# fab-jul/imgcomp-cvpr

Hardware: AMD Instinct MI355X
Metric: Megapixels/s encode+pc-logits (and decode) per node (higher is better)
Workload: dtype f32

## Files before the change

imgcomp_cvpr_amd/csrc/conv_mfma.hip:

```cpp
#include "internal.h"

typedef float f32x16 __attribute__((ext_vector_type(16)));
typedef float f32x4 __attribute__((ext_vector_type(4)));

#define GKC 8

struct GArgs {
    const float* x; const float* scale; const float* shift; float* y;
    int N, IH, IW;
    int GH, GW;
    int OH, OW, OS;
    int Cout, relu;
    int tiles_x, tiles_y;
    int ncot;
    unsigned long long* prof;
};

__global__ void pack_conv_mfma_kernel(const float* __restrict__ w, float* __restrict__ out, int KW, int Cin, int Cout,
                                      int transposed, int NTY, int NTX, int NCOT, int kyb, int kys, int kxb, int kxs,
                                      int total) {
    const int idx = blockIdx.x * 256 + threadIdx.x;
    if (idx >= total) return;
    const int j = idx & 3, l = (idx >> 2) & 63;
    int r = idx >> 8;
    const int n = r % NCOT; r /= NCOT;
    const int NT = NTY * NTX;
    const int t = r % NT, c = r / NT;
    const int ty = t / NTX, tx = t % NTX;
    const int ky = kyb + kys * ty, kx = kxb + kxs * tx;
    const int ci = GKC * c + 2 * j + (l >> 5), co = 32 * n + (l & 31);
    float v = 0.f;
    if (co < Cout)
        v = transposed ? w[(((size_t)ky * KW + kx) * Cout + co) * Cin + ci]
                       : w[(((size_t)ky * KW + kx) * Cin + ci) * Cout + co];
    out[idx] = v;
}

struct GPhase { const float* wp; int oy0, ox0, py, px; };

template <int NTY, int NTX, int PS, int WK, int TR, int TC, int CPC = 1>
struct GGeo {
    static constexpr int ROWS = (TR - 1) * PS + NTY, COLS = (TC - 1) * PS + NTX;
    static constexpr int S = COLS, CS = ROWS * COLS, CHUNK = GKC * WK * CS * CPC;
    static constexpr int NST = (CHUNK + 255) / 256;
    static constexpr int LDSF = 2 * NST * 256;
    static_assert(NST <= 32, "in-bounds mask is 32 bits");
};

template <int NTY, int NTX, int PS, int CIN, int WM, int WN, int WK, int PT, int TR, int TC, int RD, bool KEEP = false, bool X1 = false, int CPC = 1>
__device__ __forceinline__ void conv_mfma_body(const GArgs& a, const GPhase& ph, float* __restrict__ lds, f32x16* keep = nullptr) {
#ifdef CM_PROF
    const unsigned long long cm_t0 = __builtin_amdgcn_s_memtime();
#endif
    using G = GGeo<NTY, NTX, PS, WK, TR, TC, CPC>;
    constexpr int NT = NTY * NTX;
    constexpr int NCH = CIN / (GKC * WK * CPC);
    static_assert(CPC == 1 || WK == 1, "several channel groups per chunk: whole-K waves only");
    static_assert(CIN % (GKC * WK * CPC) == 0, "Cin multiple of the chunk");
    constexpr int S = G::S, CS = G::CS, CHUNK = G::CHUNK, NST = G::NST;
    static_assert(WM * WN * WK == 4, "4 waves per work-group");
    static_assert(TR * TC == 32 * PT * WN, "tile = PT accumulator tiles per wave x WN pixel groups");
    static_assert(NT % RD == 0 && RD >= 3, "ring depth must divide the tap count");
    static_assert(CIN % (GKC * WK) == 0, "Cin multiple of 8 * WK");
    static_assert(WK == 1 || (16 % WK == 0 && WM * WN * WK * PT * 16 * 64 <= G::LDSF), "reduction scratch fits in the staging buffers");

    const int tid = threadIdx.x, lane = tid & 63, wave = tid >> 6;
    const int wm = wave % WM, wn = (wave / WM) % WN, wk = wave / (WM * WN);
    int b = ic_xcd_run(blockIdx.x, gridDim.x);
    const int tx_ = b % a.tiles_x; b /= a.tiles_x;
    const int ty_ = b % a.tiles_y; const int n = b / a.tiles_y;
    const int cot = blockIdx.y * WM + wm;
    const int ncot = a.ncot;
    const int gx0 = tx_ * TC, gy0 = ty_ * TR;
    const int IHW = a.IH * a.IW;
    const float* __restrict__ xin = a.x + (size_t)n * CIN * IHW;

    int goff[NST];
    unsigned inb = 0;
    const int iy0 = gy0 * PS + ph.oy0, ix0 = gx0 * PS + ph.ox0;
#pragma unroll
    for (int i = 0; i < NST; ++i) {
        const int e = tid + 256 * i;
        const int ci = e / CS, rem = e - ci * CS;
        const int rr = rem / S, cc = rem - rr * S;
        const int iy = iy0 + rr, ix = ix0 + cc;
        const bool ok = (e < CHUNK) && iy >= 0 && iy < a.IH && ix >= 0 && ix < a.IW;
        goff[i] = ok ? ci * IHW + iy * a.IW + ix : 0;
        inb |= (ok ? 1u : 0u) << i;
    }
    const int j = lane & 31, kh = lane >> 5;
    int boff[PT];
#pragma unroll
    for (int p = 0; p < PT; ++p) {
        const int q = 32 * (PT * wn + p) + j;
        boff[p] = (GKC * wk + kh) * CS + (q / TC) * PS * S + (q % TC) * PS;
    }
    const int cot_u = __builtin_amdgcn_readfirstlane(cot), wk_u = __builtin_amdgcn_readfirstlane(wk);
    const __amdgpu_buffer_rsrc_t wr = __builtin_amdgcn_make_buffer_rsrc(
        (void*)ph.wp, 0, (CIN / GKC) * NT * ncot * 256 * 4, 0x00020000);
    const unsigned wlane = (unsigned)lane * 16u;
    const int wstep = ncot * 1024;
    const int cstep = NT * wstep;
    auto wload = [&](int c8, int t) -> f32x4 {
        return __builtin_bit_cast(f32x4, __builtin_amdgcn_raw_buffer_load_b128(wr, wlane, c8 * cstep + t * wstep + cot_u * 1024, 0));
    };

    f32x16 acc[PT];
#pragma unroll
    for (int p = 0; p < PT; ++p)
#pragma unroll
        for (int r = 0; r < 16; ++r) acc[p][r] = 0.f;

    constexpr int RPW = 16 / WK;
    float bsc[RPW], bsh[RPW];
    {
        const __amdgpu_buffer_rsrc_t scr = __builtin_amdgcn_make_buffer_rsrc((void*)a.scale, 0, a.Cout * 4, 0x00020000);
        const __amdgpu_buffer_rsrc_t shr = __builtin_amdgcn_make_buffer_rsrc((void*)a.shift, 0, a.Cout * 4, 0x00020000);
#pragma unroll
        for (int rr = 0; rr < RPW; ++rr) {
            const int r = (WK > 1 ? wk * RPW : 0) + rr;
            const unsigned co4 = (unsigned)(32 * cot + (r & 3) + 8 * (r >> 2) + 4 * (lane >> 5)) * 4u;
            bsc[rr] = __builtin_bit_cast(float, __builtin_amdgcn_raw_buffer_load_b32(scr, co4, 0, 0));
            bsh[rr] = __builtin_bit_cast(float, __builtin_amdgcn_raw_buffer_load_b32(shr, co4, 0, 0));
        }
    }
    f32x4 ring[RD];
#pragma unroll
    for (int t = 0; t < RD - 2; ++t) ring[t] = wload(wk_u, t);
    static_assert(!X1 || (PT == 1 && WM == 1 && WN == 1), "extra channel: one pixel tile per wave");
    const int cotx_u = X1 ? (a.Cout - 1) / 32 : 0;
    const unsigned xlane = (unsigned)(lane >> 5) * 512u;
    auto xload = [&](int c8, int t) -> f32x4 {
        return __builtin_bit_cast(f32x4, __builtin_amdgcn_raw_buffer_load_b128(wr, xlane, c8 * cstep + t * wstep + cotx_u * 1024, 0));
    };
    f32x4 xring[X1 ? RD : 1];
    float accx = 0.f;
    if constexpr (X1) {
#pragma unroll
        for (int t = 0; t < RD - 2; ++t) xring[t] = xload(wk_u, t);
    }
#pragma unroll
    for (int i = 0; i < NST; ++i) {
        const float v = xin[goff[i]];
        lds[tid + 256 * i] = ((inb >> i) & 1) ? v : 0.f;
    }
    __syncthreads();
#ifdef CM_PROF
    const unsigned long long cm_t1 = __builtin_amdgcn_s_memtime();
#endif

    for (int c = 0; c < NCH; ++c) {
        const bool more = c + 1 < NCH;
        float st[NST];
        if (more) {
            const float* xc = xin + (size_t)(c + 1) * GKC * WK * CPC * IHW;
#pragma unroll
            for (int i = 0; i < NST; ++i) st[i] = xc[goff[i]];
        }
        const float* __restrict__ L = lds + (c & 1) * (NST * 256);
        const int c8 = c * WK * CPC + wk_u, c8n = more ? (c + 1) * WK * CPC + wk_u : c8;
        constexpr int NU = CPC * NT;
        float bq[2][4][PT];
#pragma unroll
        for (int ks = 0; ks < 4; ++ks)
#pragma unroll
            for (int p = 0; p < PT; ++p) bq[0][ks][p] = L[boff[p] + 2 * ks * CS];
#pragma unroll
        for (int u = 0; u < NU; ++u) {
            {
                const int un = u + RD - 2;
                if (un < NU) ring[un % RD] = wload(c8 + un / NT, un % NT);
                else ring[un % RD] = wload(c8n + (un - NU) / NT, (un - NU) % NT);
                if constexpr (X1) {
                    if (un < NU) xring[un % RD] = xload(c8 + un / NT, un % NT);
                    else xring[un % RD] = xload(c8n + (un - NU) / NT, (un - NU) % NT);
                }
            }
            if (u + 1 < NU) {
                const int tn = (u + 1) % NT, gn = (u + 1) / NT;
                const int tapoff = (tn / NTX) * S + (tn % NTX) + 8 * gn * CS;
#pragma unroll
                for (int ks = 0; ks < 4; ++ks)
#pragma unroll
                    for (int p = 0; p < PT; ++p) bq[(u + 1) & 1][ks][p] = L[boff[p] + 2 * ks * CS + tapoff];
            }
#pragma unroll
            for (int ks = 0; ks < 4; ++ks) {
                const float av = ring[u % RD][ks];
#pragma unroll
                for (int p = 0; p < PT; ++p)
                    acc[p] = __builtin_amdgcn_mfma_f32_32x32x2f32(av, bq[u & 1][ks][p], acc[p], 0, 0, 0);
                if constexpr (X1) asm volatile("v_fmac_f32 %0, %1, %2" : "+v"(accx) : "v"(xring[u % RD][ks]), "v"(bq[u & 1][ks][0]));
            }
#pragma unroll
            for (int i = 0; i < 4 * PT; ++i) {
                __builtin_amdgcn_sched_group_barrier(0x008, 1, 0);
                if (i == 0) __builtin_amdgcn_sched_group_barrier(0x020, 1, 0);
                if (X1 && i == 1) __builtin_amdgcn_sched_group_barrier(0x020, 1, 0);
                if (X1) __builtin_amdgcn_sched_group_barrier(0x002, 1, 0);
                if (u + 1 < NU) __builtin_amdgcn_sched_group_barrier(0x100, 1, 0);
            }
            __builtin_amdgcn_sched_barrier(0);
        }
        if (more) {
            float* __restrict__ Ln = lds + ((c & 1) ^ 1) * (NST * 256);
#pragma unroll
            for (int i = 0; i < NST; ++i) Ln[tid + 256 * i] = ((inb >> i) & 1) ? st[i] : 0.f;
        }
        asm volatile("s_waitcnt lgkmcnt(0)" ::: "memory");
        __builtin_amdgcn_s_barrier();
    }

#ifdef CM_PROF
    const unsigned long long cm_t2 = __builtin_amdgcn_s_memtime();
#endif
    float* __restrict__ y = a.y;
    const size_t OHW = (size_t)a.OH * a.OW;
    const size_t cbase = ((size_t)n * a.Cout + 32 * cot + 4 * kh) * OHW;
    if (WK > 1) {
        float* red = lds + (size_t)((wm * WN + wn) * WK) * (PT * 16 * 64);
#pragma unroll
        for (int p = 0; p < PT; ++p)
#pragma unroll
            for (int r = 0; r < 16; ++r) red[(size_t)((wk * PT + p) * 16 + r) * 64 + lane] = acc[p][r];
        __syncthreads();
#pragma unroll
        for (int p = 0; p < PT; ++p)
#pragma unroll
            for (int rr = 0; rr < RPW; ++rr) {
                const int r = wk * RPW + rr;
                float sum = 0.f;
#pragma unroll
                for (int k2 = 0; k2 < WK; ++k2) sum += red[(size_t)((k2 * PT + p) * 16 + r) * 64 + lane];
                acc[p][rr] = sum;
            }
    }
    if constexpr (X1) {
        const float half_sum = accx + __shfl_xor(accx, 32);
        if (WK > 1) {
            __syncthreads();
            if (lane < 32) lds[wk * 32 + lane] = half_sum;
            __syncthreads();
        }
        if (wk == 0 && lane < 32) {
            float sum = WK > 1 ? 0.f : half_sum;
            if (WK > 1) {
#pragma unroll
                for (int k2 = 0; k2 < WK; ++k2) sum += lds[k2 * 32 + lane];
            }
            const int cx = a.Cout - 1;
            const int q = lane, gy = gy0 + q / TC, gx = gx0 + q % TC;
            if (gy < a.GH && gx < a.GW) {
                float v = fmaf(sum, a.scale[cx], a.shift[cx]);
                if (a.relu) v = fmaxf(v, 0.f);
                y[((size_t)n * a.Cout + cx) * OHW + (size_t)(gy * a.OS + ph.py) * a.OW + (gx * a.OS + ph.px)] = v;
            }
        }
    }
    if constexpr (KEEP) {
        static_assert(!KEEP || WK == 1, "paired phases: whole-K waves");
#pragma unroll
        for (int p = 0; p < PT; ++p)
#pragma unroll
            for (int r = 0; r < 16; ++r) {
                float v = fmaf(acc[p][r], bsc[r], bsh[r]);
                keep[p][r] = a.relu ? fmaxf(v, 0.f) : v;
            }
        return;
    }
#pragma unroll
    for (int p = 0; p < PT; ++p) {
        const int q = 32 * (PT * wn + p) + j;
        const int gy = gy0 + q / TC, gx = gx0 + q % TC;
        if (gy < a.GH && gx < a.GW) {
            const size_t pix = cbase + (size_t)(gy * a.OS + ph.py) * a.OW + (gx * a.OS + ph.px);
#pragma unroll
            for (int rr = 0; rr < RPW; ++rr) {
                const int r = (WK > 1 ? wk * RPW : 0) + rr;
                const int crow = (r & 3) + 8 * (r >> 2);
                const int co = 32 * cot + crow + 4 * kh;
                if (co < (X1 ? a.Cout - 1 : a.Cout)) {
                    float v = fmaf(acc[p][rr], bsc[rr], bsh[rr]);
                    if (a.relu) v = fmaxf(v, 0.f);
                    y[pix + (size_t)crow * OHW] = v;
                }
            }
        }
    }
#ifdef CM_PROF
    if (a.prof && lane == 0) {
        unsigned long long* d = a.prof + 4 * (((size_t)blockIdx.y * gridDim.x + blockIdx.x) * 4 + wave);
        d[0] = cm_t0; d[1] = cm_t1; d[2] = cm_t2; d[3] = __builtin_amdgcn_s_memtime();
    }
#endif
}

template <int NTY, int NTX, int PS, int CIN, int WM, int WN, int WK, int PT, int TR, int TC, int RD, int CPC = 1>
__global__ __launch_bounds__(256) void conv_mfma_kernel(const GArgs a, const GPhase ph) {
    __shared__ float lds[GGeo<NTY, NTX, PS, WK, TR, TC, CPC>::LDSF];
    conv_mfma_body<NTY, NTX, PS, CIN, WM, WN, WK, PT, TR, TC, RD, false, false, CPC>(a, ph, lds);
}

template <int NTY, int NTX, int PS, int CIN, int WM, int WN, int WK, int PT, int TR, int TC, int RD>
__global__ __launch_bounds__(256) void conv_mfma_x1_kernel(const GArgs a, const GPhase ph) {
    __shared__ float lds[GGeo<NTY, NTX, PS, WK, TR, TC>::LDSF];
    conv_mfma_body<NTY, NTX, PS, CIN, WM, WN, WK, PT, TR, TC, RD, false, true>(a, ph, lds);
}

struct GPhases4 { GPhase p[4]; };
template <int CIN, int WM, int WN, int PT, int TR, int TC>
__global__ __launch_bounds__(256) void deconv5_mfma_kernel(const GArgs a, const GPhases4 ph) {
    __shared__ float lds[GGeo<3, 3, 1, 1, TR, TC>::LDSF];
    switch (blockIdx.z) {
        case 0: conv_mfma_body<2, 2, 1, CIN, WM, WN, 1, PT, TR, TC, 4>(a, ph.p[0], lds); break;
        case 1: conv_mfma_body<2, 3, 1, CIN, WM, WN, 1, PT, TR, TC, 3>(a, ph.p[1], lds); break;
        case 2: conv_mfma_body<3, 2, 1, CIN, WM, WN, 1, PT, TR, TC, 3>(a, ph.p[2], lds); break;
        default: conv_mfma_body<3, 3, 1, CIN, WM, WN, 1, PT, TR, TC, 3>(a, ph.p[3], lds); break;
    }
}

typedef float f32x2g __attribute__((ext_vector_type(2)));
template <int CIN, int WM, int WN, int PT, int TR, int TC, int CPC>
__global__ __launch_bounds__(256) void deconv5_pair_kernel(const GArgs a, const GPhases4 ph) {
    __shared__ float lds[GGeo<3, 3, 1, 1, TR, TC, CPC>::LDSF];
    f32x16 v0[PT], v1[PT];
    const int py = blockIdx.z;
    if (py == 0) {
        conv_mfma_body<2, 2, 1, CIN, WM, WN, 1, PT, TR, TC, 4, true, false, CPC>(a, ph.p[0], lds, v0);
        conv_mfma_body<2, 3, 1, CIN, WM, WN, 1, PT, TR, TC, 3, true, false, CPC>(a, ph.p[1], lds, v1);
    } else {
        conv_mfma_body<3, 2, 1, CIN, WM, WN, 1, PT, TR, TC, 3, true, false, CPC>(a, ph.p[2], lds, v0);
        conv_mfma_body<3, 3, 1, CIN, WM, WN, 1, PT, TR, TC, 3, true, false, CPC>(a, ph.p[3], lds, v1);
    }
    const int lane = threadIdx.x & 63, wave = threadIdx.x >> 6;
    const int wm = wave % WM, wn = (wave / WM) % WN;
    int b = ic_xcd_run(blockIdx.x, gridDim.x);
    const int tx_ = b % a.tiles_x; b /= a.tiles_x;
    const int ty_ = b % a.tiles_y; const int n = b / a.tiles_y;
    const int cot = blockIdx.y * WM + wm;
    const int j = lane & 31, kh = lane >> 5;
    const size_t OHW = (size_t)a.OH * a.OW;
    float* __restrict__ y = a.y + ((size_t)n * a.Cout + 32 * cot + 4 * kh) * OHW;
#pragma unroll
    for (int p = 0; p < PT; ++p) {
        const int q = 32 * (PT * wn + p) + j;
        const int gy = ty_ * TR + q / TC, gx = tx_ * TC + q % TC;
        if (gy < a.GH && gx < a.GW) {
            const size_t pix = (size_t)(gy * 2 + py) * a.OW + gx * 2;
#pragma unroll
            for (int r = 0; r < 16; ++r) {
                const int crow = (r & 3) + 8 * (r >> 2);
                if (32 * cot + crow + 4 * kh < a.Cout)
                    *(f32x2g*)(y + pix + (size_t)crow * OHW) = f32x2g{v0[p][r], v1[p][r]};
            }
        }
    }
}

static unsigned long long* g_cm_prof = nullptr;
#ifdef CM_PROF
extern "C" void ic_conv2d_mfma_set_prof(unsigned lo, unsigned hi) { g_cm_prof = (unsigned long long*)(((unsigned long long)hi << 32) | lo); }
#endif
static int ncot_for(int Cout) { return ic_cdiv(Cout, 32) <= 2 ? 2 : ic_cdiv(ic_cdiv(Cout, 32), 4) * 4; }

static void phase_taps(int K, int pad, int p, int* nt, int* o0, int* kb) {
    const int k0 = (p + pad) & 1;
    const int cnt = (K - k0 + 1) / 2;
    const int kmax = k0 + 2 * (cnt - 1);
    *nt = cnt;
    *o0 = (p + pad - kmax) / 2;
    *kb = kmax;
}

static bool supported(int KH, int KW, int Cin, int Cout, int stride, int transposed) {
    if (KH == 3 && KW == 3 && stride == 2 && !transposed) return Cin == 128 && Cout <= 128;
    if (KH != 5 || KW != 5 || stride != 2) return false;
    if (!transposed) return (Cin == 64 && Cout == 128) || (Cin == 128 && Cout <= 128);
    return Cin == 128 && Cout == 64;
}

extern "C" size_t ic_conv2d_mfma_packed_floats(int KH, int KW, int Cin, int Cout, int stride, int transposed) {
    if (!supported(KH, KW, Cin, Cout, stride, transposed)) return 0;
    return (size_t)(Cin / GKC) * KH * KW * ncot_for(Cout) * 256;
}

extern "C" int ic_pack_conv2d_mfma_f32(const float* w_tf, float* w_packed, int KH, int KW, int Cin, int Cout,
                                       int stride, int transposed, ic_stream_t stream) {
    IC_CHECK_ARG(w_tf && w_packed);
    if (!supported(KH, KW, Cin, Cout, stride, transposed)) return IC_ERR_UNSUPPORTED;
    const int ncot = ncot_for(Cout), nch = Cin / GKC;
    hipStream_t st = (hipStream_t)stream;
    if (!transposed) {
        const int total = nch * KH * KW * ncot * 256;
        hipLaunchKernelGGL(pack_conv_mfma_kernel, dim3(ic_cdiv(total, 256)), dim3(256), 0, st, w_tf, w_packed, KW, Cin,
                           Cout, 0, KH, KW, ncot, 0, 1, 0, 1, total);
    } else {
        const int pad = 1;
        size_t off = 0;
        for (int py = 0; py < 2; ++py)
            for (int px = 0; px < 2; ++px) {
                int nty, ntx, oy0, ox0, kyb, kxb;
                phase_taps(KH, pad, py, &nty, &oy0, &kyb);
                phase_taps(KW, pad, px, &ntx, &ox0, &kxb);
                const int total = nch * nty * ntx * ncot * 256;
                hipLaunchKernelGGL(pack_conv_mfma_kernel, dim3(ic_cdiv(total, 256)), dim3(256), 0, st, w_tf,
                                   w_packed + off, KW, Cin, Cout, 1, nty, ntx, ncot, kyb, -2, kxb, -2, total);
                off += (size_t)total;
            }
    }
    IC_LAUNCH_CHECK();
    return IC_OK;
}

extern "C" int ic_conv2d_mfma_bn_act_f32(const float* x, const float* w_packed, const float* scale, const float* shift,
                                         float* y, int N, int Cin, int H, int W, int Cout, int KH, int KW, int stride,
                                         int transposed, int relu, ic_stream_t stream) {
    IC_CHECK_ARG(x && w_packed && scale && shift && y && N > 0 && H > 0 && W > 0);
    if (!supported(KH, KW, Cin, Cout, stride, transposed)) return IC_ERR_UNSUPPORTED;
    if ((long long)Cin * H * W >= (1ll << 31)) return IC_ERR_UNSUPPORTED;
    hipStream_t st = (hipStream_t)stream;
    const int ncot = ncot_for(Cout);
    GArgs a{};
    a.x = x; a.scale = scale; a.shift = shift; a.y = y;
    a.N = N; a.IH = H; a.IW = W; a.Cout = Cout; a.relu = relu; a.prof = g_cm_prof; a.ncot = ncot;
    if (!transposed) {
        GPhase ph{};
        ph.wp = w_packed; ph.py = 0; ph.px = 0;
        ph.oy0 = -ic_same_pad_before(H, KH, 2); ph.ox0 = -ic_same_pad_before(W, KW, 2);
        a.GH = ic_cdiv(H, 2); a.GW = ic_cdiv(W, 2); a.OH = a.GH; a.OW = a.GW; a.OS = 1;
        if (KH == 3) {
            a.tiles_x = ic_cdiv(a.GW, 16); a.tiles_y = ic_cdiv(a.GH, 2);
            hipLaunchKernelGGL((conv_mfma_kernel<3, 3, 2, 128, 1, 1, 4, 1, 2, 16, 3>),
                               dim3(a.tiles_x * a.tiles_y * N, ic_cdiv(Cout, 32)), dim3(256), 0, st, a, ph);
        } else if (Cin == 64) {
            a.tiles_x = ic_cdiv(a.GW, 16); a.tiles_y = ic_cdiv(a.GH, 2);
#ifndef CM_CPC_H2
#define CM_CPC_H2 2
#endif
            hipLaunchKernelGGL((conv_mfma_kernel<5, 5, 2, 64, 4, 1, 1, 1, 2, 16, 5, CM_CPC_H2>),
                               dim3(a.tiles_x * a.tiles_y * N, ncot / 4), dim3(256), 0, st, a, ph);
        } else {
            a.tiles_x = ic_cdiv(a.GW, 16); a.tiles_y = ic_cdiv(a.GH, 2);
            if (Cout % 32 == 1 && Cout > 1)
                hipLaunchKernelGGL((conv_mfma_x1_kernel<5, 5, 2, 128, 1, 1, 4, 1, 2, 16, 5>),
                                   dim3(a.tiles_x * a.tiles_y * N, (Cout - 1) / 32), dim3(256), 0, st, a, ph);
            else
                hipLaunchKernelGGL((conv_mfma_kernel<5, 5, 2, 128, 1, 1, 4, 1, 2, 16, 5>),
                                   dim3(a.tiles_x * a.tiles_y * N, ic_cdiv(Cout, 32)), dim3(256), 0, st, a, ph);
        }
    } else {
        a.GH = H; a.GW = W; a.OH = 2 * H; a.OW = 2 * W; a.OS = 2;
        const int pad = 1, nch = Cin / GKC;
        GPhases4 ph{};
        size_t off = 0;
        for (int py = 0; py < 2; ++py)
            for (int px = 0; px < 2; ++px) {
                int nty, ntx, kyb, kxb;
                GPhase& g = ph.p[py * 2 + px];
                phase_taps(KH, pad, py, &nty, &g.oy0, &kyb);
                phase_taps(KW, pad, px, &ntx, &g.ox0, &kxb);
                g.wp = w_packed + off; g.py = py; g.px = px;
                off += (size_t)nch * nty * ntx * ncot * 256;
            }
        a.tiles_x = ic_cdiv(a.GW, 16); a.tiles_y = ic_cdiv(a.GH, 4);
#ifdef CM_UNPAIRED
        hipLaunchKernelGGL((deconv5_mfma_kernel<128, 2, 2, 1, 4, 16>),
                           dim3(a.tiles_x * a.tiles_y * N, ncot / 2, 4), dim3(256), 0, st, a, ph);
#else
#ifndef CM_CPC_H12
#define CM_CPC_H12 2
#endif
        hipLaunchKernelGGL((deconv5_pair_kernel<128, 2, 2, 1, 4, 16, CM_CPC_H12>),
                           dim3(a.tiles_x * a.tiles_y * N, ncot / 2, 2), dim3(256), 0, st, a, ph);
#endif
    }
    IC_LAUNCH_CHECK();
    return IC_OK;
}
```

imgcomp_cvpr_amd/csrc/internal.h:

```cpp
#pragma once
#include "common.h"

struct ConvArgs {
    const float* x; const float* w; const float* scale; const float* shift;
    const float* res1; const float* res2; float* y;
    const float* in_mean; const float* in_std; const float* out_mean; const float* out_std;
    int N, Cin, H, W, Cout, OH, OW, KH, KW, stride, pt, pl, relu;
    int w_sci, w_sco;
    int tune;
    int builtin_norm;
    int out_phases;
};

int icx_conv2d(ConvArgs a, bool transposed, hipStream_t st);

int icx_deconv5_small_cout(const ConvArgs& a, hipStream_t st);

int icx_deconv5_cout3_mfma(const ConvArgs& a, hipStream_t st);

int icx_deconv3_mfma(const ConvArgs& a, hipStream_t st);

int icx_conv5s2_cin3_mfma(const ConvArgs& a, hipStream_t st);

size_t icx_pc_bwd_data_mfma_workspace(int N, int CinF, int CoutF, int OD, int OH, int OW);
int icx_pc_bwd_data_mfma(const float* g, const float* w, float* dx_raw, int N, int CinF, int CoutF, int OD, int OH, int OW,
                         const float* zero_bias, void* workspace, size_t workspace_bytes, hipStream_t st);
```

imgcomp_cvpr_amd/csrc/network.hip:

```cpp
#include "internal.h"
#include "wino_common.h"
#include <string.h>

static inline int layer_flags(int flags, int li) {
    const int n = (flags >> 12) & 0x7f;
    int f = flags & (0xfff | IC_CONV3_IN_FLIGHT(0xf) | IC_CONV3_NO_WINO4 | IC_CONV3_WINO4_BITS);
    if (n > 0 && li >= n) f &= ~IC_CONV3_LEAVE_IDLE_CUS;
    return f;
}

struct StackWalk {
    bool record; WnStackArgs* sa; int flags; int N, H, W; hipStream_t st; int li; int nlayers;
    int conv(const float* x, const float* const* l, const float* r1, const float* r2, float* y, int relu) {
        if (record) {
            WnStackLayer& L = sa->layers[li];
            L.x = x; L.wp = l[0] + ic_conv3x3_c128_packed_floats(); L.scale = l[1]; L.shift = l[2];
            L.res1 = r1; L.res2 = r2; L.y = y; L.relu = relu; L.pad_ = 0;
            ++li;
            return IC_OK;
        }
        const int rc = icx_conv3x3_c128_auto_next(x, l[0], l[1], l[2], r1, r2, y, N, H, W, relu, layer_flags(flags, li),
                                                  li + 1 < nlayers ? l[3] : nullptr, st);
        ++li;
        return rc;
    }
};

static int res_stack_walk(StackWalk& w, const void* const* tab, int B, float* const bufs[5], int* out_idx) {
    int cur = 0, rc;
    float* T = bufs[4];
    const float* const* t = (const float* const*)tab;
    for (int b = 0; b < B; ++b) {
        const int G = cur;
        for (int i = 0; i < 3; ++i) {
            int O = 1;
            while (O == G || O == cur) ++O;
            const float* const* l1 = t + 3 * w.li;
            if ((rc = w.conv(bufs[cur], l1, nullptr, nullptr, T, 1))) return rc;
            if ((rc = w.conv(T, l1 + 3, bufs[cur], i == 2 ? bufs[G] : nullptr, bufs[O], 0))) return rc;
            cur = O;
        }
    }
    {
        int O = 1;
        while (O == cur) ++O;
        const float* const* l1 = t + 3 * w.li;
        if ((rc = w.conv(bufs[cur], l1, nullptr, nullptr, T, 0))) return rc;
        if ((rc = w.conv(T, l1 + 3, bufs[cur], bufs[0], bufs[O], 0))) return rc;
        cur = O;
    }
    *out_idx = cur;
    return IC_OK;
}

static int stack_kernel_nb(int N, int H, int W, int nlayers, int flags) {
#ifndef IC_TUNING
    return 0;
#else
    if (!(flags & IC_CONV3_STACK_KERNEL) || (flags & (IC_CONV3_LEAVE_IDLE_CUS | IC_CONV3_PACKED_TRANSFORM))) return 0;
    if (((flags >> 19) & 0xf) >= 2) return 0;
    const int form = flags & IC_CONV3_FORM_MASK;
    if (form != IC_CONV3_AUTO && form != IC_CONV3_WINO && !(form >= IC_CONV3_WINO_SEG1 && form <= IC_CONV3_WINO_SEG3)) return 0;
    if (ic_conv3x3_c128_pick_algo(N, H, W, flags) != 1) return 0;
    long long pl[5];
    if (ic_wino3x3_c128_plan(N, H, W, flags & IC_CONV3_FORM_MASK, pl) != IC_OK) return 0;
    if (pl[0] || pl[3] || pl[4] || !pl[1]) return 0;
    return icx_wino_stack_fits(N, H, W, (int)pl[2], nlayers) ? (int)pl[2] : 0;
#endif
}

static int res_stack(const void* const* tab, int B, float* const bufs[5], int N, int H, int W, int flags,
                     hipStream_t st, int* out_idx, unsigned* sync) {
    const int nlayers = 6 * B + 2;
    const int nb = sync ? stack_kernel_nb(N, H, W, nlayers, flags) : 0;
#ifdef IC_TUNING
    if (nb) {
        WnStackArgs sa{};
        StackWalk w{true, &sa, flags, N, H, W, st, 0, nlayers};
        int rc = res_stack_walk(w, tab, B, bufs, out_idx);
        if (rc) return rc;
        sa.flags = sync; sa.N = N; sa.H = H; sa.W = W; sa.grows = ic_cdiv(H, 4); sa.gcols = ic_cdiv(W, 32);
        sa.nlayers = nlayers; sa.xcd_runs = (flags & IC_CONV3_NO_XCD_RUNS) ? 0 : 1;
        return icx_wino_stack_launch(sa, nb, st);
    }
#endif
    (void)nb;
    StackWalk w{false, nullptr, flags, N, H, W, st, 0, nlayers};
    return res_stack_walk(w, tab, B, bufs, out_idx);
}

static size_t ae_ws_floats(int N, int H, int W, int C) {
    const size_t hw = (size_t)H * W;
    return (size_t)N * (5 * 8 * hw + 16 * hw + (size_t)(C + 1) * hw / 64);
}
static size_t ae_sync_offset(int N, int H, int W, int C) { return (ae_ws_floats(N, H, W, C) * sizeof(float) + 255) & ~(size_t)255; }

extern "C" size_t ic_ae_workspace_bytes(int N, int H, int W, int C) {
    if (N <= 0 || H <= 0 || W <= 0 || C <= 0) return 0;
    return ae_sync_offset(N, H, W, C) + WN_STACK_SYNC_BYTES;
}
extern "C" size_t ic_ae_sync_pos_bytes(int N, int H, int W, int C) {
    if (N <= 0 || H <= 0 || W <= 0 || C <= 0) return 0;
    return ae_sync_offset(N, H, W, C);
}

static void carve(void* ws, int N, int H, int W, float* bufs[5], float** half, float** bott) {
    const size_t hw = (size_t)H * W;
    float* p = (float*)ws;
    for (int i = 0; i < 5; ++i) { bufs[i] = p; p += (size_t)N * 8 * hw; }
    *half = p; p += (size_t)N * 16 * hw;
    *bott = p;
}

extern "C" size_t ic_ae_res_stack_workspace_bytes(int N, int H, int W) {
    return N > 0 && H > 0 && W > 0 ? (size_t)5 * N * 128 * H * W * sizeof(float) + WN_STACK_SYNC_BYTES : 0;
}
extern "C" size_t ic_ae_res_stack_sync_pos_bytes(int N, int H, int W) {
    return N > 0 && H > 0 && W > 0 ? (size_t)5 * N * 128 * H * W * sizeof(float) : 0;
}
extern "C" int ic_ae_res_stack_f32(const float* x, const void* const* tab, int B, float* y, int N, int H, int W,
                                   void* workspace, size_t workspace_bytes, int flags, ic_stream_t stream) {
    IC_CHECK_ARG(x && tab && y && workspace && N > 0 && H > 0 && W > 0 && B >= 0);
    if (workspace_bytes < ic_ae_res_stack_workspace_bytes(N, H, W)) return IC_ERR_WORKSPACE;
    for (int i = 0; i < 3 * (6 * B + 2); ++i) IC_CHECK_ARG(tab[i] != nullptr);
    hipStream_t st = (hipStream_t)stream;
    const size_t n = (size_t)N * 128 * H * W;
    float* bufs[5];
    for (int i = 0; i < 5; ++i) bufs[i] = (float*)workspace + i * n;
    hipError_t e = hipMemcpyAsync(bufs[0], x, n * sizeof(float), hipMemcpyDeviceToDevice, st);
    if (e != hipSuccess) return (int)e;
    int o, rc;
    if ((rc = res_stack(tab, B, bufs, N, H, W, flags, st, &o, (unsigned*)((char*)workspace + ic_ae_res_stack_sync_pos_bytes(N, H, W))))) return rc;
    e = hipMemcpyAsync(y, bufs[o], n * sizeof(float), hipMemcpyDeviceToDevice, st);
    return e == hipSuccess ? IC_OK : (int)e;
}

static bool edge_layers_wino4(int N, int H4, int W4, int flags) {
    if (!(flags & IC_CONV5_BOTH_PACKED) || (flags & IC_CONV5_NO_WINO4) || !ic_wino4_conv5s2_supported(N, H4, W4)) return false;
    if (flags & IC_CONV5_WINO4) return true;
    return ic_conv3x3_c128_pick_form(N, H4, W4, flags) == 2 || ic_wino4_conv5s2_workgroups(N, H4, W4, 0) >= 160;
}
extern "C" size_t ic_conv5s2_both_packed_floats(int transposed) {
    return ic_conv2d_mfma_packed_floats(5, 5, transposed ? 128 : 64, transposed ? 64 : 128, 2, transposed ? 1 : 0) + ic_wino4_conv5s2_packed_floats();
}
extern "C" int ic_pack_conv5s2_both_f32(const float* w_tf, float* w_packed, int transposed, ic_stream_t stream) {
    IC_CHECK_ARG(w_tf && w_packed);
    const int tr = transposed ? 1 : 0, cin = tr ? 128 : 64, cout = tr ? 64 : 128;
    const int rc = ic_pack_conv2d_mfma_f32(w_tf, w_packed, 5, 5, cin, cout, 2, tr, stream);
    if (rc != IC_OK) return rc;
    return ic_pack_wino4_conv5s2_f32(w_tf, w_packed + ic_conv2d_mfma_packed_floats(5, 5, cin, cout, 2, tr), tr, stream);
}

extern "C" int ic_ae_encode_f32(const float* x, const void* const* tab, int B, int C, int L, int heatmap_on,
                                int normalize_on, float* heatmap, float* z, float* qsoft, float* qhard, float* qbar,
                                int64_t* symbols, int N, int H, int W,
                                void* workspace, size_t workspace_bytes, int flags, ic_stream_t stream) {
    IC_CHECK_ARG(x && tab && workspace && N > 0 && H > 0 && W > 0 && B >= 0 && C > 0 && L > 0);
    if (H % 8 || W % 8) return IC_ERR_UNSUPPORTED;
    if (workspace_bytes < ic_ae_workspace_bytes(N, H, W, C)) return IC_ERR_WORKSPACE;
    const int nconv = 6 * B + 2;
    for (int i = 0; i < 3 * (nconv + 3) + 1; ++i) IC_CHECK_ARG(tab[i] != nullptr);
    hipStream_t st = (hipStream_t)stream;
    float* bufs[5]; float* half; float* bott;
    carve(workspace, N, H, W, bufs, &half, &bott);
    int rc;
    const float* const* t = (const float* const*)tab;
    ConvArgs a{};
    a.x = x; a.w = t[0]; a.scale = t[1]; a.shift = t[2]; a.y = half;
    a.N = N; a.Cin = 3; a.H = H; a.W = W; a.Cout = 64; a.KH = 5; a.KW = 5; a.stride = 2; a.relu = 1;
    a.builtin_norm = normalize_on ? 1 : 0;
    rc = IC_ERR_UNSUPPORTED;
    if (edge_layers_wino4(N, H / 4, W / 4, flags)) {
        a.out_phases = 1;
        rc = icx_conv2d(a, false, st);
        if (rc == IC_OK)
            rc = ic_wino4_conv5s2_c64_c128_bn_act_f32(half, t[3] + ic_conv2d_mfma_packed_floats(5, 5, 64, 128, 2, 0), t[4], t[5], bufs[0],
                                                      N, H / 4, W / 4, 1, flags, stream);
        else if (rc != IC_ERR_UNSUPPORTED) return rc;
        a.out_phases = 0;
    }
    if (rc == IC_ERR_UNSUPPORTED) {
        if ((rc = icx_conv2d(a, false, st))) return rc;
        rc = ic_conv2d_mfma_bn_act_f32(half, t[3], t[4], t[5], bufs[0], N, 64, H / 2, W / 2, 128, 5, 5, 2, 0, 1, st);
    }
    if (rc) return rc;
    int o;
    if ((rc = res_stack(tab + 6, B, bufs, N, H / 4, W / 4, flags, st, &o, (unsigned*)((char*)workspace + ae_sync_offset(N, H, W, C))))) return rc;
    const float* const* tb = t + 6 + 3 * nconv;
    const int Cb = C + (heatmap_on ? 1 : 0);
    if ((rc = ic_conv2d_mfma_bn_act_f32(bufs[o], tb[0], tb[1], tb[2], bott, N, 128, H / 4, W / 4, Cb, 5, 5, 2, 0, 0, st)))
        return rc;
    const float* centers = tb[3];
    if (heatmap_on)
        return ic_heatmap_quantize_f32(bott, centers, L, 1.0f, heatmap, z, qsoft, qhard, qbar, symbols,
                                       N, C, H / 8, W / 8, stream);
    const long long cnt = (long long)N * C * (H / 8) * (W / 8);
    if (z) {
        hipError_t e = hipMemcpyAsync(z, bott, cnt * sizeof(float), hipMemcpyDeviceToDevice, st);
        if (e != hipSuccess) return (int)e;
    }
    if (qbar) return IC_ERR_UNSUPPORTED;
    if (!qsoft && !qhard && !symbols) return IC_OK;
    return ic_quantize_f32(bott, centers, L, 1.0f, qsoft, qhard, symbols, cnt, stream);
}

extern "C" int ic_ae_decode_f32(const float* q, const void* const* tab, int B, int C, int normalize_on,
                                float* x_out, int N, int H, int W,
                                void* workspace, size_t workspace_bytes, int flags, ic_stream_t stream) {
    IC_CHECK_ARG(q && tab && x_out && workspace && N > 0 && H > 0 && W > 0 && B >= 0 && C > 0);
    if (H % 8 || W % 8) return IC_ERR_UNSUPPORTED;
    if (workspace_bytes < ic_ae_workspace_bytes(N, H, W, C)) return IC_ERR_WORKSPACE;
    const int nconv = 6 * B + 2;
    for (int i = 0; i < 3 * (nconv + 3); ++i) IC_CHECK_ARG(tab[i] != nullptr);
    hipStream_t st = (hipStream_t)stream;
    float* bufs[5]; float* half; float* bott;
    carve(workspace, N, H, W, bufs, &half, &bott);
    int rc;
    const float* const* t = (const float* const*)tab;
    ConvArgs a{};
    a.x = q; a.w = t[0]; a.scale = t[1]; a.shift = t[2]; a.y = bufs[0];
    a.N = N; a.Cin = C; a.H = H / 8; a.W = W / 8; a.Cout = 128; a.KH = 3; a.KW = 3; a.relu = 1;
    if ((rc = icx_conv2d(a, true, st))) return rc;
    int o;
    if ((rc = res_stack(tab + 3, B, bufs, N, H / 4, W / 4, flags, st, &o, (unsigned*)((char*)workspace + ae_sync_offset(N, H, W, C))))) return rc;
    const float* const* th = t + 3 + 3 * nconv;
    rc = IC_ERR_UNSUPPORTED;
    if (edge_layers_wino4(N, H / 4, W / 4, flags))
        rc = ic_wino4_deconv5s2_c128_c64_bn_act_f32(bufs[o], th[0] + ic_conv2d_mfma_packed_floats(5, 5, 128, 64, 2, 1), th[1], th[2], half,
                                                    N, H / 4, W / 4, 1, flags, stream);
    if (rc == IC_ERR_UNSUPPORTED)
        rc = ic_conv2d_mfma_bn_act_f32(bufs[o], th[0], th[1], th[2], half, N, 128, H / 4, W / 4, 64, 5, 5, 2, 1, 1, st);
    if (rc) return rc;
    a = ConvArgs{};
    a.x = half; a.w = th[3]; a.scale = th[4]; a.shift = th[5]; a.y = x_out;
    a.N = N; a.Cin = 64; a.H = H / 2; a.W = W / 2; a.Cout = 3; a.KH = 5; a.KW = 5; a.relu = 0;
    a.builtin_norm = normalize_on ? 2 : 4;
    return icx_conv2d(a, true, st);
}

extern "C" int ic_abi_version(void) { return IC_ABI_VERSION; }

extern "C" const char* ic_strerror(int code) {
    switch (code) {
        case IC_OK: return "ok";
        case IC_ERR_ARG: return "invalid argument (null pointer or non-positive extent)";
        case IC_ERR_UNSUPPORTED: return "unsupported shape or option";
        case IC_ERR_WORKSPACE: return "workspace too small";
        default: return code > 0 ? hipGetErrorString((hipError_t)code) : "unknown error";
    }
}

struct CrcTab { uint32_t t[8][256]; };
static constexpr CrcTab make_crc_tab() {
    CrcTab r{};
    for (uint32_t i = 0; i < 256; ++i) {
        uint32_t c = i;
        for (int k = 0; k < 8; ++k) c = (c & 1) ? (c >> 1) ^ 0x82F63B78u : c >> 1;
        r.t[0][i] = c;
    }
    for (uint32_t i = 0; i < 256; ++i)
        for (int t = 1; t < 8; ++t) r.t[t][i] = (r.t[t - 1][i] >> 8) ^ r.t[0][r.t[t - 1][i] & 0xff];
    return r;
}
static constexpr CrcTab g_crc = make_crc_tab();
#define g_crc_tab g_crc.t

extern "C" uint32_t ic_crc32c(const void* data, size_t n, uint32_t crc) {
    const unsigned char* p = (const unsigned char*)data;
    uint32_t c = crc ^ 0xFFFFFFFFu;
    while (n >= 8) {
        uint32_t lo, hi;
        memcpy(&lo, p, 4); memcpy(&hi, p + 4, 4);
        lo ^= c;
        c = g_crc_tab[7][lo & 0xff] ^ g_crc_tab[6][(lo >> 8) & 0xff] ^ g_crc_tab[5][(lo >> 16) & 0xff] ^ g_crc_tab[4][lo >> 24] ^
            g_crc_tab[3][hi & 0xff] ^ g_crc_tab[2][(hi >> 8) & 0xff] ^ g_crc_tab[1][(hi >> 16) & 0xff] ^ g_crc_tab[0][hi >> 24];
        p += 8; n -= 8;
    }
    while (n--) c = g_crc_tab[0][(c ^ *p++) & 0xff] ^ (c >> 8);
    return c ^ 0xFFFFFFFFu;
}

extern "C" int ic_stream_create_cu_range(int first_cu, int n_cus, ic_stream_t* stream) {
    IC_CHECK_ARG(stream && first_cu >= 0 && n_cus > 0);
    int dev = 0, ncu = 0;
    hipError_t e = hipGetDevice(&dev);
    if (e != hipSuccess) return (int)e;
    e = hipDeviceGetAttribute(&ncu, hipDeviceAttributeMultiprocessorCount, dev);
    if (e != hipSuccess) return (int)e;
    if (first_cu + n_cus > ncu || ncu > 1024) return IC_ERR_UNSUPPORTED;
    uint32_t words[32] = {0};
    for (int b = first_cu; b < first_cu + n_cus; ++b) words[b / 32] |= 1u << (b % 32);
    hipStream_t s;
    e = hipExtStreamCreateWithCUMask(&s, (uint32_t)ic_cdiv(ncu, 32), words);
    if (e != hipSuccess) return (int)e;
    *stream = (ic_stream_t)s;
    return IC_OK;
}
extern "C" int ic_stream_destroy(ic_stream_t stream) { return stream ? (int)hipStreamDestroy((hipStream_t)stream) : IC_ERR_ARG; }

extern "C" int ic_event_create(void** ev) {
    IC_CHECK_ARG(ev);
    hipEvent_t e;
    hipError_t r = hipEventCreate(&e);
    if (r != hipSuccess) return (int)r;
    *ev = (void*)e;
    return IC_OK;
}
extern "C" int ic_event_destroy(void* ev) { return ev ? (int)hipEventDestroy((hipEvent_t)ev) : IC_ERR_ARG; }
extern "C" int ic_event_record(void* ev, ic_stream_t stream) {
    IC_CHECK_ARG(ev);
    return (int)hipEventRecord((hipEvent_t)ev, (hipStream_t)stream);
}
extern "C" int ic_event_elapsed_ms(void* start, void* stop, float* ms) {
    IC_CHECK_ARG(start && stop && ms);
    hipError_t r = hipEventSynchronize((hipEvent_t)stop);
    if (r != hipSuccess) return (int)r;
    return (int)hipEventElapsedTime(ms, (hipEvent_t)start, (hipEvent_t)stop);
}
```

imgcomp_cvpr_amd/csrc/quantize.hip:

```cpp
#include "common.h"

#define IC_MAX_L 16
#define HARD_SIGMA 1e7f

__device__ __forceinline__ void quantize_one(float z, const float* c, int L, float sigma,
                                             float& qsoft, float& qhard, int& sym) {
    float d[IC_MAX_L];
    float lmax_soft = -INFINITY, lmax_hard = -INFINITY;
    int best = 0;
#pragma unroll
    for (int j = 0; j < IC_MAX_L; ++j) {
        if (j < L) {
            const float t = fabsf(z - c[j]);
            d[j] = __fmul_rn(t, t);
            const float lh = __fmul_rn(-HARD_SIGMA, d[j]);
            if (lh > lmax_hard) { lmax_hard = lh; best = j; }
            lmax_soft = fmaxf(lmax_soft, __fmul_rn(-sigma, d[j]));
        }
    }
    float num = 0.f, den = 0.f;
#pragma unroll
    for (int j = 0; j < IC_MAX_L; ++j) {
        if (j < L) {
            const float e = expf(__fmul_rn(-sigma, d[j]) - lmax_soft);
            den += e;
        }
    }
#pragma unroll
    for (int j = 0; j < IC_MAX_L; ++j) {
        if (j < L) {
            const float e = expf(__fmul_rn(-sigma, d[j]) - lmax_soft);
            num += __fmul_rn(e / den, c[j]);
        }
    }
    qsoft = num;
    qhard = c[best];
    sym = best;
}

__global__ __launch_bounds__(256) void quantize_dev_centers_kernel(
        const float* __restrict__ z, const float* __restrict__ centers, int L, float sigma,
        float* __restrict__ qsoft, float* __restrict__ qhard, int64_t* __restrict__ symbols, long long count) {
    float c[IC_MAX_L];
#pragma unroll
    for (int j = 0; j < IC_MAX_L; ++j) c[j] = j < L ? centers[j] : 0.f;
    for (long long i = (long long)blockIdx.x * 256 + threadIdx.x; i < count; i += (long long)gridDim.x * 256) {
        float qs, qh; int s;
        quantize_one(z[i], c, L, sigma, qs, qh, s);
        if (qsoft) qsoft[i] = qs;
        if (qhard) qhard[i] = qh;
        if (symbols) symbols[i] = s;
    }
}

__global__ __launch_bounds__(256) void heatmap_quantize_kernel(
        const float* __restrict__ bn, const float* __restrict__ centers, int L, float sigma,
        float* __restrict__ heatmap, float* __restrict__ zout, float* __restrict__ qsoft,
        float* __restrict__ qhard, float* __restrict__ qbar, int64_t* __restrict__ symbols,
        int N, int C, int hw) {
    float c[IC_MAX_L];
#pragma unroll
    for (int j = 0; j < IC_MAX_L; ++j) c[j] = j < L ? centers[j] : 0.f;
    const long long count = (long long)N * C * hw;
    for (long long i = (long long)blockIdx.x * 256 + threadIdx.x; i < count; i += (long long)gridDim.x * 256) {
        const int p = (int)(i % hw);
        const long long t = i / hw;
        const int ch = (int)(t % C);
        const long long n = t / C;
        const float* b = bn + n * (long long)(C + 1) * hw;
        const float z0 = b[p];
        const float zc = b[(long long)(ch + 1) * hw + p];
        const float h2 = __fmul_rn(1.0f / (1.0f + expf(-z0)), (float)C);
        const float m = fmaxf(fminf(h2 - (float)ch, 1.0f), 0.0f);
        const float z = __fmul_rn(m, zc);
        float qs, qh; int s;
        quantize_one(z, c, L, sigma, qs, qh, s);
        if (heatmap) heatmap[i] = m;
        if (zout) zout[i] = z;
        if (qsoft) qsoft[i] = qs;
        if (qhard) qhard[i] = qh;
        if (qbar) qbar[i] = qs + (qh - qs);
        if (symbols) symbols[i] = s;
    }
}

static int grid_for(long long count) {
    long long g = (count + 255) / 256;
    return (int)(g < 1 ? 1 : (g > 2048 ? 2048 : g));
}

extern "C" int ic_quantize_f32(const float* z, const float* centers, int L, float sigma,
                               float* qsoft, float* qhard, int64_t* symbols, long long count, ic_stream_t stream) {
    IC_CHECK_ARG(z && centers && count > 0);
    if (L < 1 || L > IC_MAX_L) return IC_ERR_UNSUPPORTED;
    hipLaunchKernelGGL(quantize_dev_centers_kernel, dim3(grid_for(count)), dim3(256), 0, (hipStream_t)stream,
                       z, centers, L, sigma, qsoft, qhard, symbols, count);
    IC_LAUNCH_CHECK();
    return IC_OK;
}

extern "C" int ic_heatmap_quantize_f32(const float* bottleneck, const float* centers, int L, float sigma,
                                       float* heatmap, float* z, float* qsoft, float* qhard, float* qbar,
                                       int64_t* symbols, int N, int C, int h, int w, ic_stream_t stream) {
    IC_CHECK_ARG(bottleneck && centers && N > 0 && C > 0 && h > 0 && w > 0);
    if (L < 1 || L > IC_MAX_L) return IC_ERR_UNSUPPORTED;
    const long long count = (long long)N * C * h * w;
    hipLaunchKernelGGL(heatmap_quantize_kernel, dim3(grid_for(count)), dim3(256), 0, (hipStream_t)stream,
                       bottleneck, centers, L, sigma, heatmap, z, qsoft, qhard, qbar, symbols, N, C, h * w);
    IC_LAUNCH_CHECK();
    return IC_OK;
}
```

Baseline: 243.2.

## Fuse heatmap quantiser into the bottleneck conv epilogue

Adds a split-K MFMA conv kernel variant for the encoder's final 5x5 stride-2 conv whose epilogue applies the heatmap mask and quantisation in registers and LDS. It writes heatmap, z, qsoft, qhard, qbar and symbols directly, so the C+1 channel bottleneck tensor is no longer written out and re-read by a separate quantize kernel. In the non-heatmap path the conv now writes straight into z, replacing a device-to-device copy. The cost is a heavier epilogue, with per-thread center loads and exp-based softmax inside the conv kernel, and a hardcoded tile configuration that only supports C=32.

Result: no change. 243.0 (-0.1%).

```diff
diff --git a/imgcomp_cvpr_amd/csrc/conv_mfma.hip b/imgcomp_cvpr_amd/csrc/conv_mfma.hip
--- a/imgcomp_cvpr_amd/csrc/conv_mfma.hip
+++ b/imgcomp_cvpr_amd/csrc/conv_mfma.hip
@@ -1,4 +1,5 @@
 #include "internal.h"
+#include "quantize_core.h"
 
 typedef float f32x16 __attribute__((ext_vector_type(16)));
 typedef float f32x4 __attribute__((ext_vector_type(4)));
@@ -38,6 +39,8 @@
 
 struct GPhase { const float* wp; int oy0, ox0, py, px; };
 
+struct GQuant { const float* centers; int L; float sigma; QuantOut out; };
+
 template <int NTY, int NTX, int PS, int WK, int TR, int TC, int CPC = 1>
 struct GGeo {
     static constexpr int ROWS = (TR - 1) * PS + NTY, COLS = (TC - 1) * PS + NTX;
@@ -47,8 +50,11 @@
     static_assert(NST <= 32, "in-bounds mask is 32 bits");
 };
 
-template <int NTY, int NTX, int PS, int CIN, int WM, int WN, int WK, int PT, int TR, int TC, int RD, bool KEEP = false, bool X1 = false, int CPC = 1>
-__device__ __forceinline__ void conv_mfma_body(const GArgs& a, const GPhase& ph, float* __restrict__ lds, f32x16* keep = nullptr) {
+template <int NTY, int NTX, int PS, int CIN, int WM, int WN, int WK, int PT, int TR, int TC, int RD, bool KEEP = false, bool X1 = false, int CPC = 1,
+          bool QZ = false>
+__device__ __forceinline__ void conv_mfma_body(const GArgs& a, const GPhase& ph, float* __restrict__ lds, f32x16* keep = nullptr,
+                                               const GQuant* qz = nullptr) {
+    static_assert(!QZ || (X1 && WK > 1 && !KEEP), "quantiser epilogue: the split-K form with the extra channel");
 #ifdef CM_PROF
     const unsigned long long cm_t0 = __builtin_amdgcn_s_memtime();
 #endif
@@ -240,6 +246,13 @@
         if (WK > 1) {
             __syncthreads();
             if (lane < 32) lds[wk * 32 + lane] = half_sum;
+            if constexpr (QZ) {
+                if (wk == 0 && lane < 32) {
+                    float v = fmaf(acc[0][0], bsc[0], bsh[0]);
+                    if (a.relu) v = fmaxf(v, 0.f);
+                    lds[WK * 32 + lane] = v;
+                }
+            }
             __syncthreads();
         }
         if (wk == 0 && lane < 32) {
@@ -253,6 +266,13 @@
             if (gy < a.GH && gx < a.GW) {
                 float v = fmaf(sum, a.scale[cx], a.shift[cx]);
                 if (a.relu) v = fmaxf(v, 0.f);
+                if constexpr (QZ) {
+                    float qc[IC_MAX_L];
+#pragma unroll
+                    for (int k2 = 0; k2 < IC_MAX_L; ++k2) qc[k2] = k2 < qz->L ? qz->centers[k2] : 0.f;
+                    heatmap_quantize_one(lds[WK * 32 + lane], v, cx - 1, cx, qc, qz->L, qz->sigma, qz->out,
+                                         ((long long)n * cx + (cx - 1)) * (long long)OHW + (long long)gy * a.OW + gx);
+                } else
                 y[((size_t)n * a.Cout + cx) * OHW + (size_t)(gy * a.OS + ph.py) * a.OW + (gx * a.OS + ph.px)] = v;
             }
         }
@@ -266,6 +286,28 @@
                 float v = fmaf(acc[p][r], bsc[r], bsh[r]);
                 keep[p][r] = a.relu ? fmaxf(v, 0.f) : v;
             }
+        return;
+    }
+    if constexpr (QZ) {
+        const int gy = gy0 + j / TC, gx = gx0 + j % TC;
+        if (gy < a.GH && gx < a.GW) {
+            const int C = a.Cout - 1;
+            float qc[IC_MAX_L];
+#pragma unroll
+            for (int k2 = 0; k2 < IC_MAX_L; ++k2) qc[k2] = k2 < qz->L ? qz->centers[k2] : 0.f;
+            const float z0 = lds[WK * 32 + j];
+            const long long pix = (long long)n * C * (long long)OHW + (long long)gy * a.OW + gx;
+#pragma unroll
+            for (int rr = 0; rr < RPW; ++rr) {
+                const int r = wk * RPW + rr;
+                const int co = (r & 3) + 8 * (r >> 2) + 4 * kh;
+                if (co >= 1 && co <= C) {
+                    float v = fmaf(acc[0][rr], bsc[rr], bsh[rr]);
+                    if (a.relu) v = fmaxf(v, 0.f);
+                    heatmap_quantize_one(z0, v, co - 1, C, qc, qz->L, qz->sigma, qz->out, pix + (long long)(co - 1) * (long long)OHW);
+                }
+            }
+        }
         return;
     }
 #pragma unroll
@@ -305,6 +347,12 @@
 __global__ __launch_bounds__(256) void conv_mfma_x1_kernel(const GArgs a, const GPhase ph) {
     __shared__ float lds[GGeo<NTY, NTX, PS, WK, TR, TC>::LDSF];
     conv_mfma_body<NTY, NTX, PS, CIN, WM, WN, WK, PT, TR, TC, RD, false, true>(a, ph, lds);
+}
+
+template <int NTY, int NTX, int PS, int CIN, int WM, int WN, int WK, int PT, int TR, int TC, int RD>
+__global__ __launch_bounds__(256) void conv_mfma_x1q_kernel(const GArgs a, const GPhase ph, const GQuant qz) {
+    __shared__ float lds[GGeo<NTY, NTX, PS, WK, TR, TC>::LDSF];
+    conv_mfma_body<NTY, NTX, PS, CIN, WM, WN, WK, PT, TR, TC, RD, false, true, 1, true>(a, ph, lds, nullptr, &qz);
 }
 
 struct GPhases4 { GPhase p[4]; };
@@ -477,3 +525,23 @@
     IC_LAUNCH_CHECK();
     return IC_OK;
 }
+
+int icx_to_bn_quantize(const float* x, const float* w_packed, const float* scale, const float* shift, const float* centers, int L,
+                       float sigma, float* heatmap, float* z, float* qsoft, float* qhard, float* qbar, int64_t* symbols,
+                       int N, int H, int W, int C, hipStream_t st) {
+    IC_CHECK_ARG(x && w_packed && scale && shift && centers && N > 0 && H > 0 && W > 0);
+    if (C != 32 || L < 1 || L > IC_MAX_L || (long long)128 * H * W >= (1ll << 31)) return IC_ERR_UNSUPPORTED;
+    GArgs a{};
+    a.x = x; a.scale = scale; a.shift = shift; a.y = nullptr;
+    a.N = N; a.IH = H; a.IW = W; a.Cout = C + 1; a.relu = 0; a.prof = nullptr; a.ncot = ncot_for(C + 1);
+    GPhase ph{};
+    ph.wp = w_packed; ph.py = 0; ph.px = 0;
+    ph.oy0 = -ic_same_pad_before(H, 5, 2); ph.ox0 = -ic_same_pad_before(W, 5, 2);
+    a.GH = ic_cdiv(H, 2); a.GW = ic_cdiv(W, 2); a.OH = a.GH; a.OW = a.GW; a.OS = 1;
+    a.tiles_x = ic_cdiv(a.GW, 16); a.tiles_y = ic_cdiv(a.GH, 2);
+    GQuant qz{centers, L, sigma, QuantOut{heatmap, z, qsoft, qhard, qbar, symbols}};
+    hipLaunchKernelGGL((conv_mfma_x1q_kernel<5, 5, 2, 128, 1, 1, 4, 1, 2, 16, 5>),
+                       dim3(a.tiles_x * a.tiles_y * N, 1), dim3(256), 0, st, a, ph, qz);
+    IC_LAUNCH_CHECK();
+    return IC_OK;
+}
diff --git a/imgcomp_cvpr_amd/csrc/internal.h b/imgcomp_cvpr_amd/csrc/internal.h
--- a/imgcomp_cvpr_amd/csrc/internal.h
+++ b/imgcomp_cvpr_amd/csrc/internal.h
@@ -22,6 +22,10 @@
 
 int icx_conv5s2_cin3_mfma(const ConvArgs& a, hipStream_t st);
 
+int icx_to_bn_quantize(const float* x, const float* w_packed, const float* scale, const float* shift, const float* centers, int L,
+                       float sigma, float* heatmap, float* z, float* qsoft, float* qhard, float* qbar, int64_t* symbols,
+                       int N, int H, int W, int C, hipStream_t st);
+
 size_t icx_pc_bwd_data_mfma_workspace(int N, int CinF, int CoutF, int OD, int OH, int OW);
 int icx_pc_bwd_data_mfma(const float* g, const float* w, float* dx_raw, int N, int CinF, int CoutF, int OD, int OH, int OW,
                          const float* zero_bias, void* workspace, size_t workspace_bytes, hipStream_t st);
diff --git a/imgcomp_cvpr_amd/csrc/network.hip b/imgcomp_cvpr_amd/csrc/network.hip
--- a/imgcomp_cvpr_amd/csrc/network.hip
+++ b/imgcomp_cvpr_amd/csrc/network.hip
@@ -187,18 +187,21 @@
     int o;
     if ((rc = res_stack(tab + 6, B, bufs, N, H / 4, W / 4, flags, st, &o, (unsigned*)((char*)workspace + ae_sync_offset(N, H, W, C))))) return rc;
     const float* const* tb = t + 6 + 3 * nconv;
-    const int Cb = C + (heatmap_on ? 1 : 0);
-    if ((rc = ic_conv2d_mfma_bn_act_f32(bufs[o], tb[0], tb[1], tb[2], bott, N, 128, H / 4, W / 4, Cb, 5, 5, 2, 0, 0, st)))
-        return rc;
     const float* centers = tb[3];
-    if (heatmap_on)
+    if (heatmap_on) {
+        if (L > 16) return IC_ERR_UNSUPPORTED;
+        rc = icx_to_bn_quantize(bufs[o], tb[0], tb[1], tb[2], centers, L, 1.0f, heatmap, z, qsoft, qhard, qbar, symbols,
+                                N, H / 4, W / 4, C, st);
+        if (rc != IC_ERR_UNSUPPORTED) return rc;
+        if ((rc = ic_conv2d_mfma_bn_act_f32(bufs[o], tb[0], tb[1], tb[2], bott, N, 128, H / 4, W / 4, C + 1, 5, 5, 2, 0, 0, st)))
+            return rc;
         return ic_heatmap_quantize_f32(bott, centers, L, 1.0f, heatmap, z, qsoft, qhard, qbar, symbols,
                                        N, C, H / 8, W / 8, stream);
+    }
     const long long cnt = (long long)N * C * (H / 8) * (W / 8);
-    if (z) {
-        hipError_t e = hipMemcpyAsync(z, bott, cnt * sizeof(float), hipMemcpyDeviceToDevice, st);
-        if (e != hipSuccess) return (int)e;
-    }
+    if (z) bott = z;
+    if ((rc = ic_conv2d_mfma_bn_act_f32(bufs[o], tb[0], tb[1], tb[2], bott, N, 128, H / 4, W / 4, C, 5, 5, 2, 0, 0, st)))
+        return rc;
     if (qbar) return IC_ERR_UNSUPPORTED;
     if (!qsoft && !qhard && !symbols) return IC_OK;
     return ic_quantize_f32(bott, centers, L, 1.0f, qsoft, qhard, symbols, cnt, stream);
diff --git a/imgcomp_cvpr_amd/csrc/quantize.hip b/imgcomp_cvpr_amd/csrc/quantize.hip
--- a/imgcomp_cvpr_amd/csrc/quantize.hip
+++ b/imgcomp_cvpr_amd/csrc/quantize.hip
@@ -1,42 +1,4 @@
-#include "common.h"
-
-#define IC_MAX_L 16
-#define HARD_SIGMA 1e7f
-
-__device__ __forceinline__ void quantize_one(float z, const float* c, int L, float sigma,
-                                             float& qsoft, float& qhard, int& sym) {
-    float d[IC_MAX_L];
-    float lmax_soft = -INFINITY, lmax_hard = -INFINITY;
-    int best = 0;
-#pragma unroll
-    for (int j = 0; j < IC_MAX_L; ++j) {
-        if (j < L) {
-            const float t = fabsf(z - c[j]);
-            d[j] = __fmul_rn(t, t);
-            const float lh = __fmul_rn(-HARD_SIGMA, d[j]);
-            if (lh > lmax_hard) { lmax_hard = lh; best = j; }
-            lmax_soft = fmaxf(lmax_soft, __fmul_rn(-sigma, d[j]));
-        }
-    }
-    float num = 0.f, den = 0.f;
-#pragma unroll
-    for (int j = 0; j < IC_MAX_L; ++j) {
-        if (j < L) {
-            const float e = expf(__fmul_rn(-sigma, d[j]) - lmax_soft);
-            den += e;
-        }
-    }
-#pragma unroll
-    for (int j = 0; j < IC_MAX_L; ++j) {
-        if (j < L) {
-            const float e = expf(__fmul_rn(-sigma, d[j]) - lmax_soft);
-            num += __fmul_rn(e / den, c[j]);
-        }
-    }
-    qsoft = num;
-    qhard = c[best];
-    sym = best;
-}
+#include "quantize_core.h"
 
 __global__ __launch_bounds__(256) void quantize_dev_centers_kernel(
         const float* __restrict__ z, const float* __restrict__ centers, int L, float sigma,
@@ -62,25 +24,14 @@
 #pragma unroll
     for (int j = 0; j < IC_MAX_L; ++j) c[j] = j < L ? centers[j] : 0.f;
     const long long count = (long long)N * C * hw;
+    const QuantOut o{heatmap, zout, qsoft, qhard, qbar, symbols};
     for (long long i = (long long)blockIdx.x * 256 + threadIdx.x; i < count; i += (long long)gridDim.x * 256) {
         const int p = (int)(i % hw);
         const long long t = i / hw;
         const int ch = (int)(t % C);
         const long long n = t / C;
         const float* b = bn + n * (long long)(C + 1) * hw;
-        const float z0 = b[p];
-        const float zc = b[(long long)(ch + 1) * hw + p];
-        const float h2 = __fmul_rn(1.0f / (1.0f + expf(-z0)), (float)C);
-        const float m = fmaxf(fminf(h2 - (float)ch, 1.0f), 0.0f);
-        const float z = __fmul_rn(m, zc);
-        float qs, qh; int s;
-        quantize_one(z, c, L, sigma, qs, qh, s);
-        if (heatmap) heatmap[i] = m;
-        if (zout) zout[i] = z;
-        if (qsoft) qsoft[i] = qs;
-        if (qhard) qhard[i] = qh;
-        if (qbar) qbar[i] = qs + (qh - qs);
-        if (symbols) symbols[i] = s;
+        heatmap_quantize_one(b[p], b[(long long)(ch + 1) * hw + p], ch, C, c, L, sigma, o, i);
     }
 }
 
diff --git a/imgcomp_cvpr_amd/csrc/quantize_core.h b/imgcomp_cvpr_amd/csrc/quantize_core.h
--- /dev/null
+++ b/imgcomp_cvpr_amd/csrc/quantize_core.h
@@ -0,0 +1,59 @@
+#pragma once
+#include "common.h"
+
+#define IC_MAX_L 16
+#define HARD_SIGMA 1e7f
+
+__device__ __forceinline__ void quantize_one(float z, const float* c, int L, float sigma,
+                                             float& qsoft, float& qhard, int& sym) {
+    float d[IC_MAX_L];
+    float lmax_soft = -INFINITY, lmax_hard = -INFINITY;
+    int best = 0;
+#pragma unroll
+    for (int j = 0; j < IC_MAX_L; ++j) {
+        if (j < L) {
+            const float t = fabsf(z - c[j]);
+            d[j] = __fmul_rn(t, t);
+            const float lh = __fmul_rn(-HARD_SIGMA, d[j]);
+            if (lh > lmax_hard) { lmax_hard = lh; best = j; }
+            lmax_soft = fmaxf(lmax_soft, __fmul_rn(-sigma, d[j]));
+        }
+    }
+    float num = 0.f, den = 0.f;
+#pragma unroll
+    for (int j = 0; j < IC_MAX_L; ++j) {
+        if (j < L) {
+            const float e = expf(__fmul_rn(-sigma, d[j]) - lmax_soft);
+            den += e;
+        }
+    }
+#pragma unroll
+    for (int j = 0; j < IC_MAX_L; ++j) {
+        if (j < L) {
+            const float e = expf(__fmul_rn(-sigma, d[j]) - lmax_soft);
+            num += __fmul_rn(e / den, c[j]);
+        }
+    }
+    qsoft = num;
+    qhard = c[best];
+    sym = best;
+}
+
+struct QuantOut {
+    float* heatmap; float* z; float* qsoft; float* qhard; float* qbar; int64_t* symbols;
+};
+
+__device__ __forceinline__ void heatmap_quantize_one(float z0, float zc, int ch, int C, const float* c, int L, float sigma,
+                                                     const QuantOut& o, long long i) {
+    const float h2 = __fmul_rn(1.0f / (1.0f + expf(-z0)), (float)C);
+    const float m = fmaxf(fminf(h2 - (float)ch, 1.0f), 0.0f);
+    const float z = __fmul_rn(m, zc);
+    float qs, qh; int s;
+    quantize_one(z, c, L, sigma, qs, qh, s);
+    if (o.heatmap) o.heatmap[i] = m;
+    if (o.z) o.z[i] = z;
+    if (o.qsoft) o.qsoft[i] = qs;
+    if (o.qhard) o.qhard[i] = qh;
+    if (o.qbar) o.qbar[i] = qs + (qh - qs);
+    if (o.symbols) o.symbols[i] = s;
+}
```
